# zengxiaofei/HapHiC

Hardware: AMD Instinct MI355X
Metric: Hi-C pairs/s ingested (link-matrix build) + MCL iters/s (higher is better)
Workload: dtype u64 keys + u32 counts (ingest); f32 values, exact u64 fixed-point accumulation (MCL)

## Files before the change

haphic_amd/csrc/hhx_matrix.hip:

```cpp
#include "hhx_ingest.h"
#include "hhx_partition.h"
#include "hhx_sort.h"

using namespace hhx;

int hhx_csr_alloc_internal(i32 n_rows, i32 n_cols, i64 nnz, hhx_csr **out);

namespace {

struct RowsView {
    const i32 *fi, *fj;
    const double *val;
    __device__ __forceinline__ bool get(i64 k, i32 &a, i32 &b, u64 &ord, float &v) const {
        a = fi[k]; b = fj[k]; ord = (u64)k;
        v = (float)val[k];
        return true;
    }
};
struct RunView {
    const u64 *key, *ord_flank;
    const u32 *fl;
    __device__ __forceinline__ bool get(i64 k, i32 &a, i32 &b, u64 &ord, float &v) const {
        ord = ord_flank[k];
        if (ord == NO_ORD) return false;
// ... 168 lines not shown
    if (e != hipSuccess) { hhx_csr_free(m); return fail("dict_to_matrix: %s", hipGetErrorString(e)); }
    if (n_keys) k_fill<View><<<grid_for((u64)n_keys), 256, 0, g_stream>>>(vw, n_keys, frag_index.p, indptr.p, cursor.p, tj.p, tx.p);
    if (add_self_loops && shape) k_fill_diag<<<grid_for((u64)shape), 256, 0, g_stream>>>(shape, indptr.p, cursor.p, tj.p, tx.p);
    const i32 W = (shape + 31) / 32;
    const size_t lds = (size_t)W * 8 + 256 * 4;
    if (lds > 160 * 1024) { hhx_csr_free(m); return fail("dict_to_matrix: matrix order %d exceeds the LDS bitmap capacity", shape); }
    static int attr_set = -1;
    int attr_dev = 0;
    HHX_HIP(hipGetDevice(&attr_dev));
    if (attr_set != attr_dev) {
        (void)hipFuncSetAttribute((const void *)k_sort_rows, hipFuncAttributeMaxDynamicSharedMemorySize, 160 * 1024);
        attr_set = attr_dev;
    }
    if (shape) k_sort_rows<<<(unsigned)std::min<i64>(shape, 256 * 8), 256, lds, g_stream>>>(shape, W, indptr.p, tj.p, tx.p, m->indices.p, m->data.p);
    e = hipGetLastError();
    if (e == hipSuccess && frag_index_host)
        e = hipMemcpyAsync(frag_index_host, frag_index.p, sizeof(i32) * (size_t)n_frag, hipMemcpyDeviceToHost, g_stream);
    if (e == hipSuccess) e = hipStreamSynchronize(g_stream);
    if (e != hipSuccess) { hhx_csr_free(m); return fail("dict_to_matrix: %s", hipGetErrorString(e)); }
    if (n_linked_out) *n_linked_out = (i32)n_linked;
    *out = m;
    return 0;
}

template <class T>
int upload(DevBuf<T> &d, const T *h, size_t n) {
    if (d.alloc(n)) return 1;
    if (n) HHX_HIP(hipMemcpyAsync(d.p, h, n * sizeof(T), hipMemcpyHostToDevice, g_stream));
    return 0;
}

}

extern "C" int hhx_dict_to_matrix(i64 n_keys, const i32 *frag_i, const i32 *frag_j, const double *value, int on_device,
                                  i32 n_frag, const uint8_t *in_set_host, i32 n_rest, int add_self_loops,
                                  i32 *frag_index_host, i32 *n_linked_out, hhx_csr **out) {
    if (!out || !in_set_host || n_frag <= 0 || n_keys < 0) return fail("hhx_dict_to_matrix: bad argument");
    DevBuf<i32> sfi, sfj;
    DevBuf<double> sval;
    if (!on_device && n_keys) {
        if (upload(sfi, frag_i, (size_t)n_keys) || upload(sfj, frag_j, (size_t)n_keys) || upload(sval, value, (size_t)n_keys)) return 1;
        frag_i = sfi.p; frag_j = sfj.p; value = sval.p;
    }
    const RowsView vw{frag_i, frag_j, value};
    return build_matrix(vw, n_keys, n_frag, in_set_host, n_rest, add_self_loops, frag_index_host, n_linked_out, out);
}

namespace {

struct SrcDirected {
    typedef u64 w1_t;
    static constexpr bool MARK = false;
    static constexpr bool BATCHED = false;
    const u64 *key, *ord_flank;
    const u32 *fl;
    const unsigned char *in_set;
    __device__ __forceinline__ bool get(i64 idx, u64 &w0, u64 &w1) const {
        const i64 k = idx >> 1;
        const u64 ord = ord_flank[k];
        if (ord == NO_ORD) return false;
        const u64 ky = key[k];
        const u32 i = (u32)(ky >> ID_BITS), j = (u32)(ky & ID_MASK);
        if (!in_set[i] || !in_set[j]) return false;
        const u32 side = (u32)(idx & 1);
        const u32 a = side ? j : i, b = side ? i : j;
        w0 = ((u64)a << ID_BITS) | (u64)b;
        w1 = ((2 * ord + side) << 31) | (u64)fl[k];
        return true;
    }
};
struct DigRow {
    __device__ __forceinline__ u32 operator()(u64 w0) const { return (u32)(w0 >> ID_BITS); }
};

constexpr int PK_ID_BITS = 20, PK_CNT_BITS = 24;
constexpr u32 PK_ID_MASK = (1u << PK_ID_BITS) - 1, PK_CNT_MASK = (1u << PK_CNT_BITS) - 1;
__device__ __forceinline__ u32 xcc_id() {
#if defined(__HIP_DEVICE_COMPILE__)
    return __builtin_amdgcn_s_getreg((3 << 11) | 20) & 7u;
#else
    return 0;
#endif
}
struct SrcDirectedPacked {
    typedef NoPayload w1_t;
    static constexpr bool MARK = true;
    static constexpr bool BATCHED = true;
    static constexpr int CHUNK = 7, CHUNK_SCATTER = 4;
    const u64 *key, *ord_flank;
    const u32 *fl;
    const unsigned char *in_set;
    unsigned long long *first_pos;
    unsigned int *too_big;
    i32 n_frag;
    struct Raw { u64 ord, ky; u32 c; unsigned char si, sj; };
    static constexpr int PREFETCH = 1;
    static __device__ __forceinline__ void pin(Raw &r) { asm volatile("" : "+v"(r.ord)); asm volatile("" : "+v"(r.ky)); asm volatile("" : "+v"(r.c)); }
    __device__ __forceinline__ u32 frag_i(const Raw &r) const { return min((u32)(r.ky >> ID_BITS), (u32)n_frag - 1u); }
    __device__ __forceinline__ u32 frag_j(const Raw &r) const { return min((u32)(r.ky & ID_MASK), (u32)n_frag - 1u); }
    __device__ __forceinline__ void load1(i64 idx, Raw &r) const {
        const i64 k = idx >> 1;
        r.ord = ord_flank[k]; r.ky = key[k]; r.c = fl[k];
    }
    __device__ __forceinline__ void load2(Raw &r) const { r.si = in_set[frag_i(r)]; r.sj = in_set[frag_j(r)]; }
    __device__ __forceinline__ bool decode_marked(i64 idx, const Raw &r, u64 &w0, u64 &extra) const {
        const u32 i = (u32)(r.ky >> ID_BITS), j = (u32)(r.ky & ID_MASK);
        const u32 side = (u32)(idx & 1);
        const u32 a = side ? j : i, b = side ? i : j;
        w0 = ((u64)a << (PK_ID_BITS + PK_CNT_BITS)) | ((u64)b << PK_CNT_BITS) | (u64)(r.c & PK_CNT_MASK);
        extra = r.c > PK_CNT_MASK ? ~0ull : 2 * r.ord + side;
        return r.ord != NO_ORD && r.si && r.sj;
    }
    __device__ __forceinline__ bool decode(i64 idx, const Raw &r, u64 &w0, NoPayload &) const {
        u64 extra;
        return decode_marked(idx, r, w0, extra);
    }
    __device__ __forceinline__ bool get(i64 idx, u64 &w0, NoPayload &w1) const {
        Raw r;
        load1(idx, r);
        load2(r);
        return decode(idx, r, w0, w1);
    }
    __device__ __forceinline__ unsigned long long *my_table() const {
        return first_pos + (size_t)xcc_id() * (size_t)n_frag;
    }
    __device__ __forceinline__ u64 mark_load(i64 idx, const Raw &r) const {
        if (!first_pos) return 0;
        return __hip_atomic_load(&my_table()[(idx & 1) ? frag_j(r) : frag_i(r)], __ATOMIC_RELAXED, __HIP_MEMORY_SCOPE_AGENT);
    }
    __device__ __forceinline__ void mark_apply(u64 w0, u64 pos, u64 seen) const {
        if (!first_pos) return;
        if (pos == ~0ull) *too_big = 1u;
        else if (pos < seen) atomicMin(&my_table()[(u32)(w0 >> (PK_ID_BITS + PK_CNT_BITS)) & PK_ID_MASK], (unsigned long long)pos);
    }
};
constexpr int N_XCC = 8;
__global__ __launch_bounds__(256) void k_min_over_xcc(i32 n_frag, const unsigned long long *__restrict__ per_xcc, unsigned long long *__restrict__ out) {
    for (i32 f = blockIdx.x * blockDim.x + threadIdx.x; f < n_frag; f += gridDim.x * blockDim.x) {
        unsigned long long m = ~0ull;
#pragma unroll
        for (int x = 0; x < N_XCC; ++x) m = min(m, per_xcc[(size_t)x * n_frag + f]);
        out[f] = m;
    }
}
struct DigRowPacked {
    __device__ __forceinline__ u32 operator()(u64 w0) const { return (u32)(w0 >> (PK_ID_BITS + PK_CNT_BITS)) & PK_ID_MASK; }
};
__global__ __launch_bounds__(256) void k_len_from_base(i32 n_frag, const i64 *__restrict__ base, const i32 *__restrict__ frag_index, i32 *__restrict__ cnt) {
    for (i32 f = blockIdx.x * blockDim.x + threadIdx.x; f < n_frag; f += gridDim.x * blockDim.x)
        if (frag_index[f] >= 0) cnt[frag_index[f]] += (i32)(base[f + 1] - base[f]);
}
__global__ __launch_bounds__(256) void k_iota_u64(i64 n, u64 *out) {
    for (i64 k = (i64)blockIdx.x * blockDim.x + threadIdx.x; k < n; k += (i64)gridDim.x * blockDim.x) out[k] = (u64)k;
}
__global__ __launch_bounds__(256) void k_index_from_sorted(i64 n, const u64 *__restrict__ pos_sorted, const u64 *__restrict__ frag_sorted,
                                                           i32 *__restrict__ frag_index, unsigned int *n_linked) {
    for (i64 k = (i64)blockIdx.x * blockDim.x + threadIdx.x; k < n; k += (i64)gridDim.x * blockDim.x) {
        const bool linked = pos_sorted[k] != ~0ull;
        frag_index[frag_sorted[k]] = linked ? (i32)k : -1;
        if (linked && (k + 1 == n || pos_sorted[k + 1] == ~0ull)) *n_linked = (unsigned int)(k + 1);
    }
}
int rank_first_positions(i32 n_frag, const unsigned long long *first_pos, u64 pos_limit, i32 *frag_index, unsigned int *n_linked_dev) {
    if (n_frag <= 4096) {
        k_rank_first<<<(unsigned)((n_frag + 255) / 256), 256, 0, g_stream>>>(n_frag, first_pos, frag_index, n_linked_dev);
        HHX_LAUNCH_CHECK();
        return 0;
    }
    int bits = 1;
    while (bits < 64 && (pos_limit + 1) >> bits) ++bits;
    DevBuf<u64> iota, ks, vs;
    if (iota.alloc((size_t)n_frag) || ks.alloc((size_t)n_frag) || vs.alloc((size_t)n_frag)) return 1;
    k_iota_u64<<<(unsigned)((n_frag + 255) / 256), 256, 0, g_stream>>>(n_frag, iota.p);
    HHX_LAUNCH_CHECK();
    HHX_TRY(stable_sort_pairs_u64((const u64 *)first_pos, ks.p, iota.p, vs.p, n_frag, bits));
    k_index_from_sorted<<<(unsigned)((n_frag + 255) / 256), 256, 0, g_stream>>>(n_frag, ks.p, vs.p, frag_index, n_linked_dev);
    HHX_LAUNCH_CHECK();
    HHX_HIP(hipStreamSynchronize(g_stream));
    return 0;
}

__global__ __launch_bounds__(256) void k_row_first(i32 n_frag, const i64 *__restrict__ base, const u64 *__restrict__ w1,
                                                   unsigned long long *__restrict__ first_pos, i32 *__restrict__ row_len) {
    const int lane = lane_id();
    for (i32 a = blockIdx.x * 4 + threadIdx.x / HHX_WAVE; a < n_frag; a += gridDim.x * 4) {
        const i64 b = base[a], e = base[a + 1];
        unsigned long long m = ~0ull;
        for (i64 p = b + lane; p < e; p += HHX_WAVE) m = min(m, (unsigned long long)(w1[p] >> 31));
#pragma unroll
        for (int o = 32; o > 0; o >>= 1) m = min(m, (unsigned long long)__shfl_down((long long)m, o, HHX_WAVE));
        if (lane == 0) { first_pos[a] = m; row_len[a] = (i32)(e - b); }
    }
}
__global__ __launch_bounds__(256) void k_len_by_index(i32 n_frag, const i32 *__restrict__ frag_index, const i32 *__restrict__ row_len,
// ... 18 lines not shown
    i32 a = blockIdx.x;
    if (a >= n_frag) return;
    i32 r = frag_index[a];
    i64 b = base[a], e = r < 0 ? b : base[a + 1];
    u64 t0[EMIT_R];
#pragma unroll
    for (int u = 0; u < EMIT_R; ++u) { const i64 p = b + tid + (i64)u * EMIT_T; t0[u] = p < e ? w0[p] : 0; }
#pragma unroll
    for (int u = 0; u < EMIT_R; ++u) asm volatile("" : "+v"(t0[u]));
    for (;;) {
        const i32 an = a + gridDim.x;
        i32 rn = -1;
        i64 bn = 0, en = 0;
        u64 tn[EMIT_R];
        if (an < n_frag) { rn = frag_index[an]; bn = base[an]; en = rn < 0 ? bn : base[an + 1]; }
#pragma unroll
        for (int u = 0; u < EMIT_R; ++u) { const i64 p = bn + tid + (i64)u * EMIT_T; tn[u] = p < en ? w0[p] : 0; }
        if (r >= 0) {
            const i32 ob = indptr[r];
            for (i32 w = tid; w < W; w += EMIT_T) bitmap[w] = 0;
            i32 cc[EMIT_R];
#pragma unroll
            for (int u = 0; u < EMIT_R; ++u) { const i64 p = b + tid + (i64)u * EMIT_T; cc[u] = p < e ? frag_index[entry_col<PACKED>(t0[u])] : -1; }
            lds_barrier();
#pragma unroll
            for (int u = 0; u < EMIT_R; ++u) if (cc[u] >= 0) atomicOr(&bitmap[cc[u] >> 5], 1u << (cc[u] & 31));
            for (i64 p = b + tid + (i64)EMIT_R * EMIT_T; p < e; p += EMIT_T) { const i32 c = frag_index[entry_col<PACKED>(w0[p])]; atomicOr(&bitmap[c >> 5], 1u << (c & 31)); }
            if (self_loop && tid == 0) atomicOr(&bitmap[r >> 5], 1u << (r & 31));
            lds_barrier();
            const i32 per = (W + EMIT_T - 1) / EMIT_T, wa = min(W, tid * per), wb = min(W, wa + per);
            u32 local = 0;
            for (i32 w = wa; w < wb; ++w) local += __popc(bitmap[w]);
            u32 incl = local;
#pragma unroll
            for (int o = 1; o < HHX_WAVE; o <<= 1) {
                const u32 t = __shfl_up(incl, o, HHX_WAVE);
                if (lane >= o) incl += t;
            }
            if (lane == HHX_WAVE - 1) wsum[wave] = incl;
            lds_barrier();
            u32 run = incl - local;
            for (int w = 0; w < wave; ++w) run += wsum[w];
            for (i32 w = wa; w < wb; ++w) { prefix[w] = run; run += __popc(bitmap[w]); }
            lds_barrier();
#pragma unroll
            for (int u = 0; u < EMIT_R; ++u) asm volatile("" : "+v"(tn[u]));
            asm volatile("" : "+v"(rn)); asm volatile("" : "+v"(bn)); asm volatile("" : "+v"(en));
#pragma unroll
            for (int u = 0; u < EMIT_R; ++u)
                if (cc[u] >= 0) {
                    const i32 c = cc[u];
                    const i32 k = (i32)(prefix[c >> 5] + __popc(bitmap[c >> 5] & ((1u << (c & 31)) - 1u)));
                    oj[ob + k] = c;
                    ox[ob + k] = entry_val<PACKED>(t0[u], w1, b + tid + (i64)u * EMIT_T);
                }
            for (i64 p = b + tid + (i64)EMIT_R * EMIT_T; p < e; p += EMIT_T) {
                const u64 t = w0[p];
                const i32 c = frag_index[entry_col<PACKED>(t)];
                const i32 k = (i32)(prefix[c >> 5] + __popc(bitmap[c >> 5] & ((1u << (c & 31)) - 1u)));
                oj[ob + k] = c;
                ox[ob + k] = entry_val<PACKED>(t, w1, p);
            }
            if (self_loop && tid == 0) {
                const i32 k = (i32)(prefix[r >> 5] + __popc(bitmap[r >> 5] & ((1u << (r & 31)) - 1u)));
                oj[ob + k] = r;
                ox[ob + k] = 1.0f;
            }
            lds_barrier();
        } else {
#pragma unroll
            for (int u = 0; u < EMIT_R; ++u) asm volatile("" : "+v"(tn[u]));
            asm volatile("" : "+v"(rn)); asm volatile("" : "+v"(bn)); asm volatile("" : "+v"(en));
        }
        if (an >= n_frag) break;
        a = an; r = rn; b = bn; e = en;
#pragma unroll
        for (int u = 0; u < EMIT_R; ++u) t0[u] = tn[u];
    }
}
__global__ __launch_bounds__(256) void k_rest_rows(i32 r0, i32 shape, const i32 *__restrict__ indptr, i32 *__restrict__ oj, float *__restrict__ ox) {
    for (i32 r = r0 + blockIdx.x * blockDim.x + threadIdx.x; r < shape; r += gridDim.x * blockDim.x) { oj[indptr[r]] = r; ox[indptr[r]] = 1.0f; }
}

template <bool PACKED>
int link_matrix_partitioned(const LinkRun *run, i32 n_frag, u64 ord_limit, const uint8_t *in_set_host, i32 n_rest, int add_self_loops,
                            i32 *frag_index_host, i32 *n_linked_out, hhx_csr **out) {
    typedef typename std::conditional<PACKED, NoPayload, u64>::type W1;
    DevBuf<unsigned char> in_set;
    if (in_set.alloc((size_t)n_frag)) return 1;
    HHX_HIP(hipMemcpyAsync(in_set.p, in_set_host, (size_t)n_frag, hipMemcpyHostToDevice, g_stream));
    int row_bits = 0;
    while (((i64)1 << row_bits) < n_frag) ++row_bits;
    DevBuf<unsigned long long> first_pos;
    DevBuf<i32> frag_index, row_len;
    DevBuf<unsigned int> nl;
    if (first_pos.alloc((size_t)n_frag) || frag_index.alloc((size_t)n_frag) || nl.alloc(2)) return 1;
    HHX_HIP(hipMemsetAsync(nl.p, 0, 2 * sizeof(unsigned int), g_stream));
    Partitioned<W1> part;
    static const int level_bits = getenv("HHX_D2M_LBITS") ? atoi(getenv("HHX_D2M_LBITS")) : 9;
    if constexpr (PACKED) {
        DevBuf<unsigned long long> per_xcc;
        if (per_xcc.alloc((size_t)N_XCC * (size_t)n_frag)) return 1;
        HHX_HIP(hipMemsetAsync(per_xcc.p, 0xff, sizeof(unsigned long long) * (size_t)N_XCC * (size_t)n_frag, g_stream));
        const SrcDirectedPacked src{run->key.p, run->ord_flank.p, run->fl.p, in_set.p, nullptr, nullptr, n_frag};
        const SrcDirectedPacked marking{run->key.p, run->ord_flank.p, run->fl.p, in_set.p, per_xcc.p, nl.p + 1, n_frag};
        HHX_TRY(partition_records(src, DigRowPacked(), 2 * run->n, row_bits, level_bits, &part, "d2m", &marking));
        k_min_over_xcc<<<grid_for((u64)n_frag), 256, 0, g_stream>>>(n_frag, per_xcc.p, first_pos.p);
        HHX_LAUNCH_CHECK();
    } else {
        const SrcDirected src{run->key.p, run->ord_flank.p, run->fl.p, in_set.p};
        HHX_TRY(partition_records(src, DigRow(), 2 * run->n, row_bits, level_bits, &part, "d2m"));
        if (row_len.alloc((size_t)n_frag)) return 1;
        if (part.n_valid == 0) {
            HHX_HIP(hipMemsetAsync(first_pos.p, 0xff, sizeof(unsigned long long) * (size_t)n_frag, g_stream));
            HHX_HIP(hipMemsetAsync(row_len.p, 0, sizeof(i32) * (size_t)n_frag, g_stream));
        } else {
            KTimer kt("d2m_row_first");
            k_row_first<<<grid_for((u64)n_frag * 64), 256, 0, g_stream>>>(n_frag, part.base.p, part.w1.p, first_pos.p, row_len.p);
        }
        HHX_LAUNCH_CHECK();
    }
    { KTimer kt("d2m_rank");
    HHX_TRY(rank_first_positions(n_frag, first_pos.p, 2 * ord_limit + 1, frag_index.p, nl.p)); }
    unsigned int nl_host[2] = {0, 0};
    HHX_HIP(hipMemcpyAsync(nl_host, nl.p, sizeof nl_host, hipMemcpyDeviceToHost, g_stream));
    i64 members = 0;
    if (n_rest < 0)
        for (i32 f = 0; f < n_frag; ++f) members += in_set_host[f] != 0;
    HHX_HIP(hipStreamSynchronize(g_stream));
    if (PACKED && nl_host[1]) return -2;
    const unsigned int n_linked = nl_host[0];
    if (n_rest < 0) n_rest = (i32)(members - (i64)n_linked);
    const i64 shape64 = (i64)n_linked + n_rest;
    if (shape64 > INT32_MAX) return fail("matrix order exceeds int32");
    const i32 shape = (i32)shape64;
    DevBuf<i32> cnt, indptr;
    if (cnt.alloc((size_t)shape + 1) || indptr.alloc((size_t)shape + 2)) return 1;
    k_init_counts<<<grid_for((u64)shape + 1), 256, 0, g_stream>>>(shape, cnt.p, add_self_loops ? 1 : 0);
    if (part.n_valid) {
        if (PACKED) k_len_from_base<<<grid_for((u64)n_frag), 256, 0, g_stream>>>(n_frag, part.base.p, frag_index.p, cnt.p);
        else k_len_by_index<<<grid_for((u64)n_frag), 256, 0, g_stream>>>(n_frag, frag_index.p, row_len.p, cnt.p);
    }
    HHX_LAUNCH_CHECK();
    i64 nnz = 0;
    HHX_TRY(exclusive_scan_i32(cnt.p, indptr.p, shape, &nnz));
    hhx_csr *m = nullptr;
    HHX_TRY(hhx_csr_alloc_internal(shape, shape, nnz, &m));
    hipError_t e = hipMemcpyAsync(m->indptr.p, indptr.p, sizeof(i32) * ((size_t)shape + 1), hipMemcpyDeviceToDevice, g_stream);
    const i32 W = (shape + 31) / 32;
    const size_t lds = (size_t)W * 8 + (EMIT_T / HHX_WAVE) * 4;
    if (lds > 160 * 1024) { hhx_csr_free(m); return fail("link matrix: order %d exceeds the LDS bitmap capacity", shape); }
    static int attr_set = -1;
    int attr_dev = 0;
    HHX_HIP(hipGetDevice(&attr_dev));
    if (attr_set != attr_dev) {
        (void)hipFuncSetAttribute((const void *)k_row_emit<PACKED>, hipFuncAttributeMaxDynamicSharedMemorySize, 160 * 1024);
        attr_set = attr_dev;
    }
    if (e == hipSuccess && part.n_valid) {
        KTimer kt("d2m_emit");
        k_row_emit<PACKED><<<(unsigned)std::min<i64>(n_frag, 256 * 6), EMIT_T, lds, g_stream>>>(n_frag, W, add_self_loops, part.base.p, part.w0.p,
                                                                                          (const u64 *)part.w1.p, frag_index.p, indptr.p, m->indices.p, m->data.p);
    }
    if (e == hipSuccess && add_self_loops && shape > (i32)n_linked)
        k_rest_rows<<<grid_for((u64)(shape - (i32)n_linked)), 256, 0, g_stream>>>((i32)n_linked, shape, indptr.p, m->indices.p, m->data.p);
    if (e == hipSuccess) e = hipGetLastError();
    if (e == hipSuccess && frag_index_host)
        e = hipMemcpyAsync(frag_index_host, frag_index.p, sizeof(i32) * (size_t)n_frag, hipMemcpyDeviceToHost, g_stream);
    if (e == hipSuccess) e = hipStreamSynchronize(g_stream);
    if (e != hipSuccess) { hhx_csr_free(m); return fail("link matrix: %s", hipGetErrorString(e)); }
    if (n_linked_out) *n_linked_out = (i32)n_linked;
    *out = m;
    return 0;
}

}

int hhx_link_matrix_from_run(const LinkRun *run, i32 n_frag, u64 ord_limit, const uint8_t *in_set_host, i32 n_rest, int add_self_loops,
                             i32 *frag_index_host, i32 *n_linked_out, hhx_csr **out) {
    if (!out || !in_set_host || n_frag <= 0) return fail("hhx_ingest_link_matrix: bad argument");
    if (run && run->n && n_frag <= (1 << 20) && ord_limit <= ((u64)1 << 31) && !getenv("HHX_D2M_GENERIC")) {
        if (!getenv("HHX_D2M_WIDE")) {
            const int rc = link_matrix_partitioned<true>(run, n_frag, ord_limit, in_set_host, n_rest, add_self_loops, frag_index_host, n_linked_out, out);
            if (rc != -2) return rc;
        }
        return link_matrix_partitioned<false>(run, n_frag, ord_limit, in_set_host, n_rest, add_self_loops, frag_index_host, n_linked_out, out);
    }
    const RunView vw{run ? run->key.p : nullptr, run ? run->ord_flank.p : nullptr, run ? run->fl.p : nullptr};
    return build_matrix(vw, run ? run->n : 0, n_frag, in_set_host, n_rest, add_self_loops, frag_index_host, n_linked_out, out);
}

struct hhx_shard {
    i32 n_frag = 0;
    hhx::Partitioned<u64> part;
    hhx::DevBuf<long long> first;
    hhx::DevBuf<i32> row_len;
    hhx::DevBuf<u64> out_w0, out_w1;
    hhx::DevBuf<unsigned char> in_set;
};

namespace {

constexpr long long SHARD_NONE = INT64_MAX;

__global__ __launch_bounds__(256) void k_first_signed(i32 n_frag, const unsigned long long *__restrict__ first_pos, long long *__restrict__ out) {
    for (i32 f = blockIdx.x * blockDim.x + threadIdx.x; f < n_frag; f += gridDim.x * blockDim.x)
        out[f] = first_pos[f] == ~0ull ? SHARD_NONE : (long long)first_pos[f];
}
__global__ __launch_bounds__(256) void k_len_by_row(i32 n_frag, const i32 *__restrict__ frag_index, const i32 *__restrict__ row_len,
                                                    i64 *__restrict__ len_by_row) {
// ... 367 lines not shown
```

haphic_amd/csrc/hhx_partition.h:

```cpp
#pragma once
#include "hhx_common.h"

namespace hhx {

constexpr int PT = 512, P_MAX_BINS = 512;
struct NoPayload {};
template <class W1> struct PartW1 { static constexpr bool HAS = true; static constexpr size_t BYTES = sizeof(W1); };
template <> struct PartW1<NoPayload> { static constexpr bool HAS = false; static constexpr size_t BYTES = 0; };
template <class W1> struct PartTile { static constexpr int ITEMS = !PartW1<W1>::HAS ? 14 : (sizeof(W1) == 4 ? 8 : 7), TILE = PT * ITEMS; };

struct PartLevel {
    int total_bits;
    int shift;
    int lds_bits;
};

template <class W1>
struct SrcRecs {
    typedef W1 w1_t;
    static constexpr bool MARK = false;
    static constexpr bool BATCHED = true;
    static constexpr int CHUNK = 16, CHUNK_SCATTER = 16, PREFETCH = 2;
    const u64 *w0;
    const W1 *w1;
    struct Raw { u64 a; W1 b; };
    static __device__ __forceinline__ void pin(Raw &r) {
        asm volatile("" : "+v"(r.a));
        if constexpr (PartW1<W1>::HAS) asm volatile("" : "+v"(r.b));
    }
    __device__ __forceinline__ void load1(i64 idx, Raw &r) const {
        r.a = w0[idx];
        if constexpr (PartW1<W1>::HAS) r.b = w1[idx];
    }
    __device__ __forceinline__ void load2(Raw &) const {}
    __device__ __forceinline__ bool decode(i64, const Raw &r, u64 &a, W1 &b) const {
        a = r.a;
        if constexpr (PartW1<W1>::HAS) b = r.b;
        return true;
    }
    __device__ __forceinline__ bool get(i64 idx, u64 &a, W1 &b) const {
        a = w0[idx];
        if constexpr (PartW1<W1>::HAS) b = w1[idx];
        return true;
    }
};

template <class Src, class Dig>
__device__ __forceinline__ u32 tile_group(const Src &src, const Dig &dig, i64 first, i64 n, const PartLevel &L) {
    if (L.shift + L.lds_bits >= L.total_bits) return 0;
    u64 w0; typename Src::w1_t w1;
    (void)src.get(first < n ? first : n - 1, w0, w1);
    return (dig(w0) >> L.shift) >> L.lds_bits;
}

template <class Src, class Dig>
__global__ __launch_bounds__(PT) void k_part_count(Src src, Dig dig, i64 n, PartLevel L, unsigned long long *__restrict__ ghist) {
    constexpr int P_ITEMS = PartTile<typename Src::w1_t>::ITEMS, P_TILE = PartTile<typename Src::w1_t>::TILE;
    __shared__ u32 hist[P_MAX_BINS];
    __shared__ u32 s_grp;
    const int tid = threadIdx.x, nb = 1 << L.lds_bits;
    for (int t = tid; t < nb; t += PT) hist[t] = 0;
    u32 cur = 0xffffffffu;
    const i64 n_tiles = (n + P_TILE - 1) / P_TILE;
    for (i64 tile = blockIdx.x; tile < n_tiles; tile += gridDim.x) {
        const i64 base = tile * P_TILE;
        if (tid == 0) s_grp = tile_group(src, dig, base, n, L);
        lds_barrier();
        const u32 tg = s_grp;
        if (tg != cur) {
            if (cur != 0xffffffffu)
                for (int t = tid; t < nb; t += PT) {
                    if (hist[t]) atomicAdd(&ghist[((u64)cur << L.lds_bits) | (u64)t], (unsigned long long)hist[t]);
                    hist[t] = 0;
                }
            cur = tg;
            lds_barrier();
        }
        if constexpr (Src::BATCHED) {
            constexpr int CH = Src::CHUNK < P_ITEMS ? Src::CHUNK : P_ITEMS;
#pragma unroll
            for (int h = 0; h < P_ITEMS; h += CH) {
                typename Src::Raw raw[CH];
                u64 seen[CH];
#pragma unroll
                for (int k = 0; k < CH; ++k)
                    if (h + k < P_ITEMS) {
                        const i64 idx = base + (i64)(h + k) * PT + tid;
                        src.load1(idx < n ? idx : n - 1, raw[k]);
                    }
#pragma unroll
                for (int k = 0; k < CH; ++k)
                    if (h + k < P_ITEMS) {
                        src.load2(raw[k]);
                        if constexpr (Src::MARK) seen[k] = src.mark_load(base + (i64)(h + k) * PT + tid, raw[k]);
                    }
#pragma unroll
                for (int k = 0; k < CH; ++k)
                    if (h + k < P_ITEMS) {
                        const i64 idx = base + (i64)(h + k) * PT + tid;
                        u64 w0, extra = 0;
                        bool ok;
                        if constexpr (Src::MARK) ok = src.decode_marked(idx, raw[k], w0, extra);
                        else { typename Src::w1_t w1; ok = src.decode(idx, raw[k], w0, w1); }
                        if (idx < n && ok) {
                            if constexpr (Src::MARK) src.mark_apply(w0, extra, seen[k]);
                            const u32 d = dig(w0) >> L.shift;
                            if ((d >> L.lds_bits) == tg) atomicAdd(&hist[d & (u32)(nb - 1)], 1u);
                            else atomicAdd(&ghist[d], 1ull);
                        }
                    }
            }
        } else {
            static_assert(!Src::MARK, "a source with a side effect per record is a BATCHED one");
#pragma unroll
        for (int k = 0; k < P_ITEMS; ++k) {
            const i64 idx = base + (i64)k * PT + tid;
            u64 w0; typename Src::w1_t w1;
            if (idx < n && src.get(idx, w0, w1)) {
                const u32 d = dig(w0) >> L.shift;
                if ((d >> L.lds_bits) == tg) atomicAdd(&hist[d & (u32)(nb - 1)], 1u);
                else atomicAdd(&ghist[d], 1ull);
            }
        }
        }
        lds_barrier();
    }
    if (cur != 0xffffffffu)
        for (int t = tid; t < nb; t += PT)
            if (hist[t]) atomicAdd(&ghist[((u64)cur << L.lds_bits) | (u64)t], (unsigned long long)hist[t]);
}

template <class W1, int T>
constexpr size_t part_scatter_lds() {
    return (size_t)PartTile<W1>::ITEMS * T * (8 + PartW1<W1>::BYTES + 2) + (size_t)P_MAX_BINS * (4 + 4 + 8) + 16;
}

template <class Src, bool B = Src::BATCHED> struct PartRaw { struct type {}; static constexpr int PF = 0; };
template <class Src> struct PartRaw<Src, true> { typedef typename Src::Raw type; static constexpr int PF = Src::PREFETCH; };

template <class Src, class Dig, int T>
__global__ __launch_bounds__(T) void k_part_scatter(Src src, Dig dig, i64 n, PartLevel L, unsigned long long *__restrict__ cursor,
                                                     u64 *__restrict__ out_w0, typename Src::w1_t *__restrict__ out_w1) {
    typedef typename Src::w1_t W1;
    typedef typename PartRaw<Src>::type RawT;
    constexpr int P_ITEMS = PartTile<W1>::ITEMS, P_TILE = PartTile<W1>::ITEMS * T, PF = PartRaw<Src>::PF;
    static_assert(P_TILE <= 0x10000 && P_MAX_BINS <= 0x8000, "bin and rank of a record share one register");
    extern __shared__ __attribute__((aligned(16))) unsigned char smem[];
    u64 *s_w0 = (u64 *)smem;
    unsigned long long *gbase = (unsigned long long *)(s_w0 + P_TILE);
    W1 *s_w1 = (W1 *)(gbase + P_MAX_BINS);
    u32 *hist = (u32 *)((unsigned char *)s_w1 + (size_t)P_TILE * PartW1<W1>::BYTES);
    u32 *lbase = hist + P_MAX_BINS;
    u32 *s_misc = lbase + P_MAX_BINS;
    unsigned short *s_bin = (unsigned short *)(s_misc + 4);
    const int tid = threadIdx.x, lane = lane_id(), wave = tid / HHX_WAVE, nb = 1 << L.lds_bits;
    __shared__ u32 wsum[T / HHX_WAVE];
    const i64 n_tiles = (n + P_TILE - 1) / P_TILE;
    if ((i64)blockIdx.x >= n_tiles) return;
    const bool later = L.shift + L.lds_bits < L.total_bits;
    for (int t = tid; t < nb; t += T) hist[t] = 0;
    lds_barrier();
    [[maybe_unused]] auto prefetch = [&](const i64 pbase, RawT (&raw)[P_ITEMS], u64 &gw) {
        if constexpr (PF > 0) {
#pragma unroll
            for (int k = 0; k < P_ITEMS; ++k) {
                const i64 idx = pbase + (i64)k * T + tid;
                src.load1(idx < n ? idx : n - 1, raw[k]);
            }
            if constexpr (PF > 1) {
#pragma unroll
                for (int k = 0; k < P_ITEMS; ++k) src.load2(raw[k]);
            }
            if (later) { W1 gw1; (void)src.get(pbase < n ? pbase : n - 1, gw, gw1); }
        }
    };
    [[maybe_unused]] auto pin = [&](RawT (&raw)[P_ITEMS], u64 &gw) {
        if constexpr (PF > 0) {
#pragma unroll
            for (int k = 0; k < P_ITEMS; ++k) Src::pin(raw[k]);
            asm volatile("" : "+v"(gw));
        }
    };
    [[maybe_unused]] RawT raw_c[P_ITEMS];
    [[maybe_unused]] u64 gw_c = 0;
    prefetch((i64)blockIdx.x * P_TILE, raw_c, gw_c);
    pin(raw_c, gw_c);
    for (i64 tile = blockIdx.x; tile < n_tiles; tile += gridDim.x) {
        const i64 base = tile * P_TILE;
        u32 tg = 0;
        if constexpr (PF > 0) { if (later) tg = (dig(gw_c) >> L.shift) >> L.lds_bits; }
        else tg = tile_group(src, dig, base, n, L);
        u64 w0[P_ITEMS];
        W1 w1[P_ITEMS];
        u32 lr[P_ITEMS];
        bool have[P_ITEMS];
        if constexpr (PF > 0) {
            constexpr int CH = PF > 1 ? P_ITEMS : (Src::CHUNK_SCATTER < P_ITEMS ? Src::CHUNK_SCATTER : P_ITEMS);
#pragma unroll
            for (int h = 0; h < P_ITEMS; h += CH) {
                if constexpr (PF == 1) {
#pragma unroll
                    for (int k = 0; k < CH; ++k)
                        if (h + k < P_ITEMS) src.load2(raw_c[h + k]);
                }
#pragma unroll
                for (int k = 0; k < CH; ++k)
                    if (h + k < P_ITEMS) {
                        const i64 idx = base + (i64)(h + k) * T + tid;
                        const bool ok = src.decode(idx, raw_c[h + k], w0[h + k], w1[h + k]);
                        have[h + k] = idx < n && ok;
                    }
            }
        } else if constexpr (Src::BATCHED) {
            constexpr int CH = Src::CHUNK_SCATTER < P_ITEMS ? Src::CHUNK_SCATTER : P_ITEMS;
#pragma unroll
            for (int h = 0; h < P_ITEMS; h += CH) {
                RawT raw[CH];
#pragma unroll
                for (int k = 0; k < CH; ++k)
                    if (h + k < P_ITEMS) {
                        const i64 idx = base + (i64)(h + k) * T + tid;
                        src.load1(idx < n ? idx : n - 1, raw[k]);
                    }
#pragma unroll
                for (int k = 0; k < CH; ++k)
                    if (h + k < P_ITEMS) src.load2(raw[k]);
#pragma unroll
                for (int k = 0; k < CH; ++k)
                    if (h + k < P_ITEMS) {
                        const i64 idx = base + (i64)(h + k) * T + tid;
                        const bool ok = src.decode(idx, raw[k], w0[h + k], w1[h + k]);
                        have[h + k] = idx < n && ok;
                    }
            }
        }
#pragma unroll
        for (int k = 0; k < P_ITEMS; ++k) {
            const i64 idx = base + (i64)k * T + tid;
            lr[k] = 0xffffffffu;
            if constexpr (!Src::BATCHED) have[k] = idx < n && src.get(idx, w0[k], w1[k]);
            if (have[k]) {
                const u32 d = dig(w0[k]) >> L.shift;
                if ((d >> L.lds_bits) == tg) {
// ... 13 lines not shown
        const u32 c = tid < nb ? hist[tid] : 0;
        if (tid < nb) hist[tid] = 0;
        u32 incl = c;
#pragma unroll
        for (int o = 1; o < HHX_WAVE; o <<= 1) {
            const u32 v = __shfl_up(incl, o, HHX_WAVE);
            if (lane >= o) incl += v;
        }
        if (lane == HHX_WAVE - 1) wsum[wave] = incl;
        lds_barrier();
        u32 woff = 0;
        for (int w = 0; w < wave; ++w) woff += wsum[w];
        unsigned long long gb = 0;
        if (tid < nb) {
            lbase[tid] = woff + incl - c;
            if (c) gb = atomicAdd(&cursor[((u64)tg << L.lds_bits) | (u64)tid], (unsigned long long)c);
        }
        if (tid == T - 1) s_misc[1] = woff + incl;
        lds_barrier();
#pragma unroll
        for (int k = 0; k < P_ITEMS; ++k)
            if (lr[k] != 0xffffffffu) {
                const u32 loc = lr[k] >> 16;
                const u32 s = lbase[loc] + (lr[k] & 0xffffu);
                s_w0[s] = w0[k];
                if constexpr (PartW1<W1>::HAS) s_w1[s] = w1[k];
                s_bin[s] = (unsigned short)loc;
            }
        if (c) gbase[tid] = gb;
        pin(raw_n, gw_n);
        lds_barrier();
        const u32 staged = s_misc[1];
        for (u32 s = tid; s < staged; s += T) {
            const u32 b = s_bin[s];
            const unsigned long long pos = gbase[b] + (s - lbase[b]);
            out_w0[pos] = s_w0[s];
            if constexpr (PartW1<W1>::HAS) out_w1[pos] = s_w1[s];
        }
        if constexpr (PF > 0) {
#pragma unroll
            for (int k = 0; k < P_ITEMS; ++k) raw_c[k] = raw_n[k];
            gw_c = gw_n;
        }
    }
}

template <class Src> constexpr int part_scatter_threads() { return PartRaw<Src>::PF == 2 ? 2 * PT : PT; }

inline i64 part_grid_cap() { const char *e = getenv("HHX_PART_GRID"); return e && atoll(e) > 0 ? atoll(e) : 256 * 4; }

void u64_copy_async(const unsigned long long *src, unsigned long long *dst, i64 n);

template <class W1>
struct Partitioned {
    DevBuf<u64> w0;
    DevBuf<W1> w1;
    DevBuf<i64> base;
    i64 n_valid = 0;
    u32 n_buckets = 1;
};

inline int part_levels(int total_bits, int max_bits, int *bits ) {
    int n = total_bits <= 0 ? 1 : (total_bits + max_bits - 1) / max_bits;
    if (n > 4) n = 4;
    int left = total_bits;
    static const bool ascending = !getenv("HHX_PART_DESC");
    for (int l = 0; l < n; ++l) {
        bits[l] = ascending ? left / (n - l) : (left + (n - l) - 1) / (n - l);
        left -= bits[l];
    }
    return n;
}

template <class Src, class Dig>
int partition_records(const Src &src, const Dig &dig, i64 n_items, int total_bits, int max_bits_per_level,
                      Partitioned<typename Src::w1_t> *out, const char *timer_prefix, const Src *count_src = nullptr,
                      const unsigned long long *hist0 = nullptr) {
    typedef typename Src::w1_t W1;
    constexpr int T1 = part_scatter_threads<Src>(), TN = part_scatter_threads<SrcRecs<W1>>();
    static int attr_dev = -1;
    int dev = 0;
    HHX_HIP(hipGetDevice(&dev));
    if (attr_dev != dev) {
        HHX_HIP(hipFuncSetAttribute((const void *)k_part_scatter<Src, Dig, T1>, hipFuncAttributeMaxDynamicSharedMemorySize, (int)part_scatter_lds<W1, T1>()));
        HHX_HIP(hipFuncSetAttribute((const void *)k_part_scatter<SrcRecs<W1>, Dig, TN>, hipFuncAttributeMaxDynamicSharedMemorySize, (int)part_scatter_lds<W1, TN>()));
        attr_dev = dev;
    }
    if (max_bits_per_level > 9) max_bits_per_level = 9;
    int bits[4];
    const int n_levels = part_levels(total_bits, max_bits_per_level, bits);
    int used = 0;
    for (int l = 0; l < n_levels; ++l) used += bits[l];
    if (used != total_bits) return fail("partition: %d bits do not fit %d levels", total_bits, n_levels);
    out->n_buckets = 1u << total_bits;
    DevBuf<u64> cur_w0, nxt_w0;
    DevBuf<W1> cur_w1, nxt_w1;
    DevBuf<i64> base;
    i64 n_cur = n_items;
    int done_bits = 0;
    char tname[64];
    for (int l = 0; l < n_levels; ++l) {
        done_bits += bits[l];
        const u32 nbk = 1u << done_bits;
        const PartLevel L{total_bits, total_bits - done_bits, bits[l]};
        DevBuf<unsigned long long> hist, cursor;
        DevBuf<i64> nbase;
        if (hist.alloc((size_t)nbk + 1) || cursor.alloc((size_t)nbk + 1) || nbase.alloc((size_t)nbk + 2)) return 1;
        HHX_HIP(hipMemsetAsync(hist.p, 0, sizeof(unsigned long long) * ((size_t)nbk + 1), g_stream));
        const i64 tile = l == 0 ? PartTile<W1>::TILE : PartTile<W1>::TILE;
        const unsigned grid = (unsigned)std::max<i64>(1, std::min<i64>((n_cur + tile - 1) / tile, part_grid_cap()));
        const SrcRecs<W1> rs{cur_w0.p, cur_w1.p};
        snprintf(tname, sizeof tname, "%s_count%d", timer_prefix, l + 1);
        { KTimer kt(tname);
        if (l == 0 && hist0) u64_copy_async(hist0, hist.p, (i64)nbk);
        else if (l == 0) k_part_count<Src, Dig><<<grid, PT, 0, g_stream>>>(count_src ? *count_src : src, dig, n_cur, L, hist.p);
        else k_part_count<SrcRecs<W1>, Dig><<<grid, PT, 0, g_stream>>>(rs, dig, n_cur, L, hist.p); }
        HHX_LAUNCH_CHECK();
        i64 n_valid = 0;
        HHX_TRY(exclusive_scan_i64((const i64 *)hist.p, nbase.p, nbk, &n_valid));
        if (l == 0) out->n_valid = n_valid;
        if (n_valid == 0) {
            out->n_valid = 0;
            out->base = std::move(nbase);
            return 0;
        }
        if (nxt_w0.alloc((size_t)n_valid) || (PartW1<W1>::HAS && nxt_w1.alloc((size_t)n_valid))) return 1;
        u64_copy_async((const unsigned long long *)nbase.p, cursor.p, (i64)nbk + 1);
        snprintf(tname, sizeof tname, "%s_scatter%d", timer_prefix, l + 1);
        { KTimer kt(tname);
        const i64 stile = (i64)PartTile<W1>::ITEMS * (l == 0 ? T1 : TN);
        const unsigned sgrid = (unsigned)std::max<i64>(1, std::min<i64>((n_cur + stile - 1) / stile, part_grid_cap()));
        if (l == 0) k_part_scatter<Src, Dig, T1><<<sgrid, T1, part_scatter_lds<W1, T1>(), g_stream>>>(src, dig, n_cur, L, cursor.p, nxt_w0.p, nxt_w1.p);
        else k_part_scatter<SrcRecs<W1>, Dig, TN><<<sgrid, TN, part_scatter_lds<W1, TN>(), g_stream>>>(rs, dig, n_cur, L, cursor.p, nxt_w0.p, nxt_w1.p); }
        HHX_LAUNCH_CHECK();
        HHX_HIP(hipStreamSynchronize(g_stream));
        cur_w0 = std::move(nxt_w0);
        cur_w1 = std::move(nxt_w1);
        base = std::move(nbase);
        n_cur = n_valid;
    }
    out->w0 = std::move(cur_w0);
    out->w1 = std::move(cur_w1);
    out->base = std::move(base);
    return 0;
}

}
```

Before: 15.64 billion.

## Pack fragment membership into bitset and stage it in LDS for d2m partition

The byte-per-fragment membership array is replaced by a host-packed u32 bitset. When the fragment count fits (up to 2^19), each count and scatter block copies the whole bitset into LDS at startup, so membership checks become LDS reads instead of two dependent global gathers per record. The host also counts members while packing, which replaces a separate loop. In exchange, every block pays an upfront bitset copy (up to 64KB), and the extra dynamic LDS in the scatter kernel may lower occupancy.

```diff
diff --git a/haphic_amd/csrc/hhx_matrix.hip b/haphic_amd/csrc/hhx_matrix.hip
--- a/haphic_amd/csrc/hhx_matrix.hip
+++ b/haphic_amd/csrc/hhx_matrix.hip
@@ -274,34 +274,58 @@
     return 0;
 #endif
 }
+constexpr i32 D2M_LDS_MAX_FRAGS = 1 << 19;
+struct PackedRawBase { u64 ord, ky; u32 c; };
+struct PackedRawWords : PackedRawBase { u32 wi, wj; };
+template <bool IN_LDS>
 struct SrcDirectedPacked {
     typedef NoPayload w1_t;
     static constexpr bool MARK = true;
     static constexpr bool BATCHED = true;
+    static constexpr bool LDS_TABLE = IN_LDS;
+    static constexpr size_t LDS_TABLE_MAX = (size_t)D2M_LDS_MAX_FRAGS / 8;
     static constexpr int CHUNK = 7, CHUNK_SCATTER = 4;
     const u64 *key, *ord_flank;
     const u32 *fl;
-    const unsigned char *in_set;
+    const u32 *in_bits;
     unsigned long long *first_pos;
     unsigned int *too_big;
     i32 n_frag;
-    struct Raw { u64 ord, ky; u32 c; unsigned char si, sj; };
+    typedef typename std::conditional<IN_LDS, PackedRawBase, PackedRawWords>::type Raw;
     static constexpr int PREFETCH = 1;
     static __device__ __forceinline__ void pin(Raw &r) { asm volatile("" : "+v"(r.ord)); asm volatile("" : "+v"(r.ky)); asm volatile("" : "+v"(r.c)); }
     __device__ __forceinline__ u32 frag_i(const Raw &r) const { return min((u32)(r.ky >> ID_BITS), (u32)n_frag - 1u); }
     __device__ __forceinline__ u32 frag_j(const Raw &r) const { return min((u32)(r.ky & ID_MASK), (u32)n_frag - 1u); }
+    size_t lds_table_bytes() const { return ((size_t)n_frag + 31) / 32 * sizeof(u32); }
+    __device__ __forceinline__ SrcDirectedPacked lds_table(void *at) const {
+        u32 *t = (u32 *)at;
+        const u32 words = ((u32)n_frag + 31u) >> 5;
+        for (u32 w = threadIdx.x; w < words; w += blockDim.x) t[w] = in_bits[w];
+        SrcDirectedPacked s = *this;
+        s.in_bits = t;
+        return s;
+    }
     __device__ __forceinline__ void load1(i64 idx, Raw &r) const {
         const i64 k = idx >> 1;
         r.ord = ord_flank[k]; r.ky = key[k]; r.c = fl[k];
     }
-    __device__ __forceinline__ void load2(Raw &r) const { r.si = in_set[frag_i(r)]; r.sj = in_set[frag_j(r)]; }
+    __device__ __forceinline__ void load2(Raw &r) const {
+        if constexpr (!IN_LDS) { r.wi = in_bits[frag_i(r) >> 5]; r.wj = in_bits[frag_j(r) >> 5]; }
+    }
+    __device__ __forceinline__ bool member(const Raw &r) const {
+        const u32 fi = frag_i(r), fj = frag_j(r);
+        u32 wi, wj;
+        if constexpr (IN_LDS) { wi = in_bits[fi >> 5]; wj = in_bits[fj >> 5]; }
+        else { wi = r.wi; wj = r.wj; }
+        return ((wi >> (fi & 31u)) & (wj >> (fj & 31u)) & 1u) != 0;
+    }
     __device__ __forceinline__ bool decode_marked(i64 idx, const Raw &r, u64 &w0, u64 &extra) const {
         const u32 i = (u32)(r.ky >> ID_BITS), j = (u32)(r.ky & ID_MASK);
         const u32 side = (u32)(idx & 1);
         const u32 a = side ? j : i, b = side ? i : j;
         w0 = ((u64)a << (PK_ID_BITS + PK_CNT_BITS)) | ((u64)b << PK_CNT_BITS) | (u64)(r.c & PK_CNT_MASK);
         extra = r.c > PK_CNT_MASK ? ~0ull : 2 * r.ord + side;
-        return r.ord != NO_ORD && r.si && r.sj;
+        return r.ord != NO_ORD && member(r);
     }
     __device__ __forceinline__ bool decode(i64 idx, const Raw &r, u64 &w0, NoPayload &) const {
         u64 extra;
@@ -486,13 +510,47 @@
     for (i32 r = r0 + blockIdx.x * blockDim.x + threadIdx.x; r < shape; r += gridDim.x * blockDim.x) { oj[indptr[r]] = r; ox[indptr[r]] = 1.0f; }
 }
 
+i64 pack_membership(const uint8_t *in_set_host, i32 n_frag, u32 *bits) {
+    const i32 n_words = (n_frag + 31) / 32;
+    for (i32 w = 0; w < n_words; ++w) bits[w] = 0;
+    i64 members = 0;
+    i32 f = 0;
+    for (; f + 8 <= n_frag; f += 8) {
+        u64 x;
+        memcpy(&x, in_set_host + f, 8);
+        const u64 y = (((x & 0x7f7f7f7f7f7f7f7full) + 0x7f7f7f7f7f7f7f7full) | x) & 0x8080808080808080ull;
+        const u32 m = (u32)(((y >> 7) * 0x0102040810204080ull) >> 56);
+        bits[f >> 5] |= m << (f & 31);
+        members += __builtin_popcount(m);
+    }
+    for (; f < n_frag; ++f)
+        if (in_set_host[f]) { bits[f >> 5] |= 1u << (f & 31); ++members; }
+    return members;
+}
+i32 d2m_lds_frags() {
+    const char *e = getenv("HHX_D2M_LDS_FRAGS");
+    if (!e || !*e) return D2M_LDS_MAX_FRAGS;
+    const long long v = atoll(e);
+    return v <= 0 ? 0 : (i32)std::min<long long>(v, D2M_LDS_MAX_FRAGS);
+}
+
 template <bool PACKED>
 int link_matrix_partitioned(const LinkRun *run, i32 n_frag, u64 ord_limit, const uint8_t *in_set_host, i32 n_rest, int add_self_loops,
                             i32 *frag_index_host, i32 *n_linked_out, hhx_csr **out) {
     typedef typename std::conditional<PACKED, NoPayload, u64>::type W1;
     DevBuf<unsigned char> in_set;
-    if (in_set.alloc((size_t)n_frag)) return 1;
-    HHX_HIP(hipMemcpyAsync(in_set.p, in_set_host, (size_t)n_frag, hipMemcpyHostToDevice, g_stream));
+    DevBuf<u32> in_bits;
+    std::vector<u32> bits_host;
+    i64 members = 0;
+    if constexpr (PACKED) {
+        bits_host.resize(((size_t)n_frag + 31) / 32);
+        members = pack_membership(in_set_host, n_frag, bits_host.data());
+        if (in_bits.alloc(bits_host.size())) return 1;
+        HHX_HIP(hipMemcpyAsync(in_bits.p, bits_host.data(), sizeof(u32) * bits_host.size(), hipMemcpyHostToDevice, g_stream));
+    } else {
+        if (in_set.alloc((size_t)n_frag)) return 1;
+        HHX_HIP(hipMemcpyAsync(in_set.p, in_set_host, (size_t)n_frag, hipMemcpyHostToDevice, g_stream));
+    }
     int row_bits = 0;
     while (((i64)1 << row_bits) < n_frag) ++row_bits;
     DevBuf<unsigned long long> first_pos;
@@ -506,9 +564,15 @@
         DevBuf<unsigned long long> per_xcc;
         if (per_xcc.alloc((size_t)N_XCC * (size_t)n_frag)) return 1;
         HHX_HIP(hipMemsetAsync(per_xcc.p, 0xff, sizeof(unsigned long long) * (size_t)N_XCC * (size_t)n_frag, g_stream));
-        const SrcDirectedPacked src{run->key.p, run->ord_flank.p, run->fl.p, in_set.p, nullptr, nullptr, n_frag};
-        const SrcDirectedPacked marking{run->key.p, run->ord_flank.p, run->fl.p, in_set.p, per_xcc.p, nl.p + 1, n_frag};
-        HHX_TRY(partition_records(src, DigRowPacked(), 2 * run->n, row_bits, level_bits, &part, "d2m", &marking));
+        if (n_frag <= d2m_lds_frags()) {
+            const SrcDirectedPacked<true> src{run->key.p, run->ord_flank.p, run->fl.p, in_bits.p, nullptr, nullptr, n_frag};
+            const SrcDirectedPacked<true> marking{run->key.p, run->ord_flank.p, run->fl.p, in_bits.p, per_xcc.p, nl.p + 1, n_frag};
+            HHX_TRY(partition_records(src, DigRowPacked(), 2 * run->n, row_bits, level_bits, &part, "d2m", &marking));
+        } else {
+            const SrcDirectedPacked<false> src{run->key.p, run->ord_flank.p, run->fl.p, in_bits.p, nullptr, nullptr, n_frag};
+            const SrcDirectedPacked<false> marking{run->key.p, run->ord_flank.p, run->fl.p, in_bits.p, per_xcc.p, nl.p + 1, n_frag};
+            HHX_TRY(partition_records(src, DigRowPacked(), 2 * run->n, row_bits, level_bits, &part, "d2m", &marking));
+        }
         k_min_over_xcc<<<grid_for((u64)n_frag), 256, 0, g_stream>>>(n_frag, per_xcc.p, first_pos.p);
         HHX_LAUNCH_CHECK();
     } else {
@@ -528,8 +592,7 @@
     HHX_TRY(rank_first_positions(n_frag, first_pos.p, 2 * ord_limit + 1, frag_index.p, nl.p)); }
     unsigned int nl_host[2] = {0, 0};
     HHX_HIP(hipMemcpyAsync(nl_host, nl.p, sizeof nl_host, hipMemcpyDeviceToHost, g_stream));
-    i64 members = 0;
-    if (n_rest < 0)
+    if (!PACKED && n_rest < 0)
         for (i32 f = 0; f < n_frag; ++f) members += in_set_host[f] != 0;
     HHX_HIP(hipStreamSynchronize(g_stream));
     if (PACKED && nl_host[1]) return -2;
diff --git a/haphic_amd/csrc/hhx_partition.h b/haphic_amd/csrc/hhx_partition.h
--- a/haphic_amd/csrc/hhx_partition.h
+++ b/haphic_amd/csrc/hhx_partition.h
@@ -1,4 +1,5 @@
 #pragma once
+#include <type_traits>
 #include "hhx_common.h"
 
 namespace hhx {
@@ -45,6 +46,16 @@
     }
 };
 
+template <class Src, class = void> struct PartLds { static constexpr bool HAS = false; static constexpr size_t MAX = 0; };
+template <class Src> struct PartLds<Src, std::void_t<decltype(Src::LDS_TABLE)>> {
+    static constexpr bool HAS = Src::LDS_TABLE;
+    static constexpr size_t MAX = HAS ? (Src::LDS_TABLE_MAX + 15) / 16 * 16 : 0;
+};
+template <class Src> inline size_t part_lds_table_bytes(const Src &src) {
+    if constexpr (PartLds<Src>::HAS) return (src.lds_table_bytes() + 15) / 16 * 16;
+    else return 0;
+}
+
 template <class Src, class Dig>
 __device__ __forceinline__ u32 tile_group(const Src &src, const Dig &dig, i64 first, i64 n, const PartLevel &L) {
     if (L.shift + L.lds_bits >= L.total_bits) return 0;
@@ -54,12 +65,18 @@
 }
 
 template <class Src, class Dig>
-__global__ __launch_bounds__(PT) void k_part_count(Src src, Dig dig, i64 n, PartLevel L, unsigned long long *__restrict__ ghist) {
+__global__ __launch_bounds__(PT) void k_part_count(Src src_arg, Dig dig, i64 n, PartLevel L, unsigned long long *__restrict__ ghist) {
     constexpr int P_ITEMS = PartTile<typename Src::w1_t>::ITEMS, P_TILE = PartTile<typename Src::w1_t>::TILE;
     __shared__ u32 hist[P_MAX_BINS];
     __shared__ u32 s_grp;
+    extern __shared__ __attribute__((aligned(16))) unsigned char count_smem[];
     const int tid = threadIdx.x, nb = 1 << L.lds_bits;
     for (int t = tid; t < nb; t += PT) hist[t] = 0;
+    Src src = src_arg;
+    if constexpr (PartLds<Src>::HAS) {
+        src = src_arg.lds_table(count_smem);
+        lds_barrier();
+    }
     u32 cur = 0xffffffffu;
     const i64 n_tiles = (n + P_TILE - 1) / P_TILE;
     for (i64 tile = blockIdx.x; tile < n_tiles; tile += gridDim.x) {
@@ -134,12 +151,14 @@
 constexpr size_t part_scatter_lds() {
     return (size_t)PartTile<W1>::ITEMS * T * (8 + PartW1<W1>::BYTES + 2) + (size_t)P_MAX_BINS * (4 + 4 + 8) + 16;
 }
+template <class W1, int T>
+constexpr size_t part_scatter_table_at() { return (part_scatter_lds<W1, T>() + 15) / 16 * 16; }
 
 template <class Src, bool B = Src::BATCHED> struct PartRaw { struct type {}; static constexpr int PF = 0; };
 template <class Src> struct PartRaw<Src, true> { typedef typename Src::Raw type; static constexpr int PF = Src::PREFETCH; };
 
 template <class Src, class Dig, int T>
-__global__ __launch_bounds__(T) void k_part_scatter(Src src, Dig dig, i64 n, PartLevel L, unsigned long long *__restrict__ cursor,
+__global__ __launch_bounds__(T) void k_part_scatter(Src src_arg, Dig dig, i64 n, PartLevel L, unsigned long long *__restrict__ cursor,
                                                      u64 *__restrict__ out_w0, typename Src::w1_t *__restrict__ out_w1) {
     typedef typename Src::w1_t W1;
     typedef typename PartRaw<Src>::type RawT;
@@ -159,6 +178,8 @@
     if ((i64)blockIdx.x >= n_tiles) return;
     const bool later = L.shift + L.lds_bits < L.total_bits;
     for (int t = tid; t < nb; t += T) hist[t] = 0;
+    Src src = src_arg;
+    if constexpr (PartLds<Src>::HAS) src = src_arg.lds_table(smem + part_scatter_table_at<W1, T>());
     lds_barrier();
     [[maybe_unused]] auto prefetch = [&](const i64 pbase, RawT (&raw)[P_ITEMS], u64 &gw) {
         if constexpr (PF > 0) {
@@ -338,7 +359,9 @@
     int dev = 0;
     HHX_HIP(hipGetDevice(&dev));
     if (attr_dev != dev) {
-        HHX_HIP(hipFuncSetAttribute((const void *)k_part_scatter<Src, Dig, T1>, hipFuncAttributeMaxDynamicSharedMemorySize, (int)part_scatter_lds<W1, T1>()));
+        HHX_HIP(hipFuncSetAttribute((const void *)k_part_scatter<Src, Dig, T1>, hipFuncAttributeMaxDynamicSharedMemorySize, (int)(part_scatter_table_at<W1, T1>() + PartLds<Src>::MAX)));
+        if constexpr (PartLds<Src>::HAS)
+            HHX_HIP(hipFuncSetAttribute((const void *)k_part_count<Src, Dig>, hipFuncAttributeMaxDynamicSharedMemorySize, (int)PartLds<Src>::MAX));
         HHX_HIP(hipFuncSetAttribute((const void *)k_part_scatter<SrcRecs<W1>, Dig, TN>, hipFuncAttributeMaxDynamicSharedMemorySize, (int)part_scatter_lds<W1, TN>()));
         attr_dev = dev;
     }
@@ -348,6 +371,8 @@
     int used = 0;
     for (int l = 0; l < n_levels; ++l) used += bits[l];
     if (used != total_bits) return fail("partition: %d bits do not fit %d levels", total_bits, n_levels);
+    const size_t table_bytes = part_lds_table_bytes(src);
+    if (table_bytes > PartLds<Src>::MAX) return fail("partition: an LDS table of %zu bytes exceeds the %zu its source declares", table_bytes, PartLds<Src>::MAX);
     out->n_buckets = 1u << total_bits;
     DevBuf<u64> cur_w0, nxt_w0;
     DevBuf<W1> cur_w1, nxt_w1;
@@ -369,7 +394,7 @@
         snprintf(tname, sizeof tname, "%s_count%d", timer_prefix, l + 1);
         { KTimer kt(tname);
         if (l == 0 && hist0) u64_copy_async(hist0, hist.p, (i64)nbk);
-        else if (l == 0) k_part_count<Src, Dig><<<grid, PT, 0, g_stream>>>(count_src ? *count_src : src, dig, n_cur, L, hist.p);
+        else if (l == 0) k_part_count<Src, Dig><<<grid, PT, table_bytes, g_stream>>>(count_src ? *count_src : src, dig, n_cur, L, hist.p);
         else k_part_count<SrcRecs<W1>, Dig><<<grid, PT, 0, g_stream>>>(rs, dig, n_cur, L, hist.p); }
         HHX_LAUNCH_CHECK();
         i64 n_valid = 0;
@@ -386,7 +411,7 @@
         { KTimer kt(tname);
         const i64 stile = (i64)PartTile<W1>::ITEMS * (l == 0 ? T1 : TN);
         const unsigned sgrid = (unsigned)std::max<i64>(1, std::min<i64>((n_cur + stile - 1) / stile, part_grid_cap()));
-        if (l == 0) k_part_scatter<Src, Dig, T1><<<sgrid, T1, part_scatter_lds<W1, T1>(), g_stream>>>(src, dig, n_cur, L, cursor.p, nxt_w0.p, nxt_w1.p);
+        if (l == 0) k_part_scatter<Src, Dig, T1><<<sgrid, T1, part_scatter_table_at<W1, T1>() + table_bytes, g_stream>>>(src, dig, n_cur, L, cursor.p, nxt_w0.p, nxt_w1.p);
         else k_part_scatter<SrcRecs<W1>, Dig, TN><<<sgrid, TN, part_scatter_lds<W1, TN>(), g_stream>>>(rs, dig, n_cur, L, cursor.p, nxt_w0.p, nxt_w1.p); }
         HHX_LAUNCH_CHECK();
         HHX_HIP(hipStreamSynchronize(g_stream));
```

Result: faster. 16.08 billion (median of 6 runs) (+2.8%).
